# lightec-xyz/bls-verify-gadget

Measured on AMD Instinct MI355X. Metric: BLS-verify witness instances/sec (full pairing circuit), higher is better.
Workload: dtype u32 (381-bit Montgomery integers mod the BLS12-381 prime as 12 x 32-bit limbs in memory, products on 14 x 28-bit limbs with 64-bit columns; SHA-256 words)

## Files before the change

### __graft_entry__.py

```python
import importlib
import os
import subprocess
import sys

ROOT = os.path.dirname(os.path.abspath(__file__))
if ROOT not in sys.path:
    sys.path.insert(0, ROOT)


def build():
    pkg = importlib.import_module("bls-verify-gadget_amd")
    pkg.build(force=False)
    subprocess.check_call(["make", "-s", "-C", os.path.join(ROOT, "oracle")])
    subprocess.check_call(["make", "-s", "-C", os.path.join(ROOT, "tests", "hostsim")])
    subprocess.check_call(["make", "-s", "-C", os.path.join(ROOT, "tests", "vgroups")])
    subprocess.check_call(["make", "-s", "-j3", "-C", os.path.join(ROOT, "tests", "devfield")])
    subprocess.check_call(["make", "-s", "-C", os.path.join(ROOT, "tests", "msg_input")])
    subprocess.check_call(["make", "-s", "-C", os.path.join(ROOT, "tests", "agg_inputs")])
    subprocess.check_call(["make", "-s", "-C", os.path.join(ROOT, "tests", "c_caller")])
    subprocess.check_call(["make", "-s", "-C", os.path.join(ROOT, "tests", "cpp_caller")])
    pkg.lib()
    for s in pkg.EXPORTED_SYMBOLS:
        getattr(pkg.lib(), s)


def smoke():
    import numpy as np
    import torch

    from tests import oracle_lib, synth

    pkg = importlib.import_module("bls-verify-gadget_amd")
    o = oracle_lib.load()
    n = 4
    pk, msg, sig, expect = synth.make_batch(o, n, seed=0x5EED)
    dev = torch.device("cuda:0")
    g = pkg.BlsSignatureVerifyGadget(n, 32, device=dev)
    res = g.verify(pkg.ParametersVar(), pkg.PublicKeyVar.new_witness(torch.from_numpy(pk.view(np.int64)).to(dev)),
                   torch.from_numpy(msg).to(dev), pkg.SignatureVar.new_witness(torch.from_numpy(sig.view(np.int64)).to(dev)))
    torch.cuda.synchronize()
    got = res.cpu().numpy().astype(bool)
    w = g.witness.cpu().numpy().view(np.uint64)
    for i in range(n):
        nw, _, r, ow = o.witness(pk[i], msg[i].tobytes(), sig[i])
        assert r == bool(got[i]) == bool(expect[i]), (i, r, got[i], expect[i])
        assert nw == w.shape[1] and np.array_equal(ow, w[i]), "witness mismatch for instance %d" % i
    print("smoke ok: %d instances, %d witnesses each, bit-exact vs oracle" % (n, w.shape[1]))


if __name__ == "__main__":
    build()
    if "--smoke" in sys.argv:
        smoke()
```

### bls-verify-gadget_amd/csrc/fp.hpp

```cpp
#pragma once
#include <stdint.h>

#if defined(__HIPCC__)
#include <hip/hip_runtime.h>
#define BLSW_HD __host__ __device__ __forceinline__
#define BLSW_HD_NOINLINE inline __host__ __device__ __noinline__
#if defined(BLSW_INLINE_CHAINS) && defined(__HIP_DEVICE_COMPILE__)
#define BLSW_FN __host__ __device__ __forceinline__
#else
#define BLSW_FN inline __host__ __device__ __noinline__
#endif
#else
#define BLSW_HD inline
#define BLSW_HD_NOINLINE inline
#define BLSW_FN inline
#endif

namespace blsw {

struct Fp {
    uint32_t l[12];
};
struct Fp2 {
    Fp c0, c1;
// ... 29 lines not shown
    Fp r;
#pragma unroll
    for (int i = 0; i < 12; i++) r.l[i] = 0;
    return r;
}
BLSW_HD Fp fp_one() {
    constexpr uint32_t R1[12] = BLSW_R1_LIMBS;
    Fp r;
#pragma unroll
    for (int i = 0; i < 12; i++) r.l[i] = R1[i];
    return r;
}
BLSW_HD bool fp_is_zero(const Fp& a) {
    uint32_t o = 0;
#pragma unroll
    for (int i = 0; i < 12; i++) o |= a.l[i];
    return o == 0;
}
BLSW_HD bool fp_eq(const Fp& a, const Fp& b) {
    uint32_t o = 0;
#pragma unroll
    for (int i = 0; i < 12; i++) o |= a.l[i] ^ b.l[i];
    return o == 0;
}
#if defined(__clang__)
BLSW_HD uint32_t addc32(uint32_t a, uint32_t b, uint32_t& carry) {
    unsigned co;
    uint32_t r = __builtin_addc(a, b, carry, &co);
    carry = co;
    return r;
}
BLSW_HD uint32_t subb32(uint32_t a, uint32_t b, uint32_t& borrow) {
    unsigned bo;
    uint32_t r = __builtin_subc(a, b, borrow, &bo);
    borrow = bo;
    return r;
}
#else
BLSW_HD uint32_t addc32(uint32_t a, uint32_t b, uint32_t& carry) {
    uint64_t x = (uint64_t)a + b + carry;
    carry = (uint32_t)(x >> 32);
    return (uint32_t)x;
}
BLSW_HD uint32_t subb32(uint32_t a, uint32_t b, uint32_t& borrow) {
    uint64_t x = (uint64_t)a - b - borrow;
    borrow = (uint32_t)(x >> 32) & 1u;
    return (uint32_t)x;
}
#endif
BLSW_HD Fp fp_cond_sub_p(const Fp& a, uint32_t top) {
    constexpr uint32_t P[12] = BLSW_P_LIMBS;
    Fp d;
    uint32_t borrow = 0;
#pragma unroll
    for (int i = 0; i < 12; i++) d.l[i] = subb32(a.l[i], P[i], borrow);
    bool ge = (top != 0) || (borrow == 0);
    Fp r;
#pragma unroll
    for (int i = 0; i < 12; i++) r.l[i] = ge ? d.l[i] : a.l[i];
    return r;
}
BLSW_HD Fp fp_add(const Fp& a, const Fp& b) {
    Fp s;
    uint32_t c = 0;
#pragma unroll
    for (int i = 0; i < 12; i++) s.l[i] = addc32(a.l[i], b.l[i], c);
    return fp_cond_sub_p(s, c);
}
BLSW_HD Fp fp_sub(const Fp& a, const Fp& b) {
    constexpr uint32_t P[12] = BLSW_P_LIMBS;
    Fp d;
    uint32_t borrow = 0;
#pragma unroll
    for (int i = 0; i < 12; i++) d.l[i] = subb32(a.l[i], b.l[i], borrow);
    uint32_t mask = 0u - borrow;
    uint32_t c = 0;
    Fp r;
#pragma unroll
    for (int i = 0; i < 12; i++) r.l[i] = addc32(d.l[i], P[i] & mask, c);
    return r;
}
BLSW_HD Fp fp_neg(const Fp& a) { return fp_sub(fp_zero(), a); }
BLSW_HD Fp fp_dbl(const Fp& a) { return fp_add(a, a); }

#if defined(__HIPCC__)
typedef uint4 blsw_u4;
#else
struct blsw_u4 {
    uint32_t x, y, z, w;
};
#endif
BLSW_HD_NOINLINE Fp fp_mul_v(blsw_u4 a0, blsw_u4 a1, blsw_u4 a2, blsw_u4 b0, blsw_u4 b1, blsw_u4 b2) {
    constexpr uint32_t P[12] = BLSW_P_LIMBS;
    const uint32_t al[12] = {a0.x, a0.y, a0.z, a0.w, a1.x, a1.y, a1.z, a1.w, a2.x, a2.y, a2.z, a2.w};
    const uint32_t bl[12] = {b0.x, b0.y, b0.z, b0.w, b1.x, b1.y, b1.z, b1.w, b2.x, b2.y, b2.z, b2.w};
    uint32_t t[13];
#pragma unroll
    for (int i = 0; i < 13; i++) t[i] = 0;
#pragma unroll
    for (int i = 0; i < 12; i++) {
        const uint32_t bi = bl[i];
        uint64_t x[12];
#pragma unroll
        for (int j = 0; j < 12; j++) x[j] = (uint64_t)al[j] * bi + t[j];
        uint32_t c = 0;
        t[0] = (uint32_t)x[0];
#pragma unroll
        for (int j = 1; j < 12; j++) t[j] = addc32((uint32_t)x[j], (uint32_t)(x[j - 1] >> 32), c);
        t[12] = addc32(t[12], (uint32_t)(x[11] >> 32), c);
        const uint32_t m = t[0] * BLSW_INV32;
#pragma unroll
        for (int j = 0; j < 12; j++) x[j] = (uint64_t)m * P[j] + t[j];
        c = 0;
#pragma unroll
        for (int j = 1; j < 12; j++) t[j - 1] = addc32((uint32_t)x[j], (uint32_t)(x[j - 1] >> 32), c);
        t[11] = addc32(t[12], (uint32_t)(x[11] >> 32), c);
        t[12] = c;
    }
    Fp r;
#pragma unroll
    for (int i = 0; i < 12; i++) r.l[i] = t[i];
    return fp_cond_sub_p(r, 0);
}
#define BLSW_P28                                                                                                                               \
    {                                                                                                                                          \
        0xfffaaabu, 0xfefffffu, 0x3ffffb9u, 0xfffeb15u, 0x6241eabu, 0xa0f6b0fu, 0xf6730d2u, 0xf38512bu, 0x4774b84u, 0x4bacd76u, 0xba7b643u, \
            0xe69a4b1u, 0x1ea397fu, 0x001a011u                                                                                                 \
    }
#define BLSW_PINV28 0xffcfffdu
BLSW_HD_NOINLINE Fp fp_mul_v28(blsw_u4 a0, blsw_u4 a1, blsw_u4 a2, blsw_u4 b0, blsw_u4 b1, blsw_u4 b2) {
    constexpr uint32_t P28[14] = BLSW_P28;
    const uint32_t M28 = 0x0fffffffu;
    const uint32_t al[12] = {a0.x, a0.y, a0.z, a0.w, a1.x, a1.y, a1.z, a1.w, a2.x, a2.y, a2.z, a2.w};
    const uint32_t bl[12] = {b0.x, b0.y, b0.z, b0.w, b1.x, b1.y, b1.z, b1.w, b2.x, b2.y, b2.z, b2.w};
    uint32_t A[14], B[14];
#pragma unroll
    for (int i = 0; i < 14; i++) {
        const int bp = 28 * i, w = bp >> 5, sh = bp & 31;
        uint32_t v = al[w] >> sh;
        if (sh > 4 && w + 1 < 12) v |= al[w + 1] << (32 - sh);
        A[i] = v & M28;
        const int bq = 28 * i - 8;
        uint32_t u;
        if (bq < 0)
            u = bl[0] << 8;
        else {
            const int wq = bq >> 5, sq = bq & 31;
            u = bl[wq] >> sq;
            if (sq > 4 && wq + 1 < 12) u |= bl[wq + 1] << (32 - sq);
        }
        B[i] = u & M28;
    }
    uint64_t t[15];
#pragma unroll
    for (int j = 0; j < 15; j++) t[j] = 0;
#pragma unroll
    for (int i = 0; i < 14; i++) {
        const uint32_t bi = B[i];
#pragma unroll
        for (int j = 0; j < 14; j++) t[j] += (uint64_t)A[j] * bi;
        const uint32_t m = ((uint32_t)t[0] * BLSW_PINV28) & M28;
#pragma unroll
        for (int j = 0; j < 14; j++) t[j] += (uint64_t)m * P28[j];
        t[1] += t[0] >> 28;
#pragma unroll
        for (int j = 0; j < 14; j++) t[j] = t[j + 1];
// ... 324 lines not shown
```

### bls-verify-gadget_amd/csrc/team.hpp

```cpp
#pragma once
#include "team_tables.hpp"
#include "tower.hpp"

namespace blsw {

#if defined(__HIP_DEVICE_COMPILE__)
typedef uint32_t team_u32x4 __attribute__((ext_vector_type(4)));
typedef __attribute__((address_space(3))) team_u32x4 team_lds_u32x4;
BLSW_HD Fp2 team_ld(const Fp2* slots, uint32_t s) {
    const team_lds_u32x4* p = (const team_lds_u32x4*)(slots + s);
    team_u32x4 v0 = p[0], v1 = p[1], v2 = p[2], v3 = p[3], v4 = p[4], v5 = p[5];
    Fp2 r;
    r.c0.l[0] = v0.x; r.c0.l[1] = v0.y; r.c0.l[2] = v0.z; r.c0.l[3] = v0.w;
    r.c0.l[4] = v1.x; r.c0.l[5] = v1.y; r.c0.l[6] = v1.z; r.c0.l[7] = v1.w;
    r.c0.l[8] = v2.x; r.c0.l[9] = v2.y; r.c0.l[10] = v2.z; r.c0.l[11] = v2.w;
    r.c1.l[0] = v3.x; r.c1.l[1] = v3.y; r.c1.l[2] = v3.z; r.c1.l[3] = v3.w;
    r.c1.l[4] = v4.x; r.c1.l[5] = v4.y; r.c1.l[6] = v4.z; r.c1.l[7] = v4.w;
    r.c1.l[8] = v5.x; r.c1.l[9] = v5.y; r.c1.l[10] = v5.z; r.c1.l[11] = v5.w;
    return r;
}
BLSW_HD void team_st(Fp2* slots, uint32_t s, const Fp2& v) {
    team_lds_u32x4* p = (team_lds_u32x4*)(slots + s);
    p[0] = team_u32x4{v.c0.l[0], v.c0.l[1], v.c0.l[2], v.c0.l[3]};
    p[1] = team_u32x4{v.c0.l[4], v.c0.l[5], v.c0.l[6], v.c0.l[7]};
    p[2] = team_u32x4{v.c0.l[8], v.c0.l[9], v.c0.l[10], v.c0.l[11]};
    p[3] = team_u32x4{v.c1.l[0], v.c1.l[1], v.c1.l[2], v.c1.l[3]};
    p[4] = team_u32x4{v.c1.l[4], v.c1.l[5], v.c1.l[6], v.c1.l[7]};
    p[5] = team_u32x4{v.c1.l[8], v.c1.l[9], v.c1.l[10], v.c1.l[11]};
}
#else
BLSW_HD Fp2 team_ld(const Fp2* slots, uint32_t s) { return slots[s]; }
BLSW_HD void team_st(Fp2* slots, uint32_t s, const Fp2& v) { slots[s] = v; }
#endif

BLSW_HD uint32_t team_lin_idx(const TeamLin& L, uint32_t k) {
    uint64_t lo = L.idx[0] | ((uint64_t)L.idx[1] << 32), hi = L.idx[2] | ((uint64_t)L.idx[3] << 32);
    uint64_t w = (k & 8) ? hi : lo;
    return (uint32_t)(w >> ((k & 7) * 8)) & 0xffu;
}
BLSW_HD Fp2 team_gather(const TeamLin& L, const Fp2* slots) {
    Fp2 acc = fp2_zero();
    uint32_t k = 0;
    const uint32_t n0 = L.n & 0x3f, n1 = (L.n >> 8) & 0xff, n2 = (L.n >> 16) & 0xff, n3 = L.n >> 24;
    const uint32_t mscale = (L.n >> 6) & 3;
    if (n0) {
        acc = team_ld(slots, team_lin_idx(L, 0));
        k = 1;
        for (; k < n0; k++) acc = fp2_add(acc, team_ld(slots, team_lin_idx(L, k)));
    }
    for (uint32_t e = k + n1; k < e; k++) acc = fp2_sub(acc, team_ld(slots, team_lin_idx(L, k)));
    if (n2 + n3) {
        Fp2 m = fp2_zero();
        for (uint32_t e = k + n2; k < e; k++) m = fp2_add(m, team_ld(slots, team_lin_idx(L, k)));
        for (uint32_t e = k + n3; k < e; k++) m = fp2_sub(m, team_ld(slots, team_lin_idx(L, k)));
        if (mscale) {
            Fp2 m3 = fp2_add(fp2_dbl(m), m);
            Fp2 m12 = fp2_dbl(fp2_dbl(m3));
            m = mscale == 2 ? fp2_dbl(m12) : m12;
        }
        acc = fp2_add(acc, fp2_mul_xi(m));
    }
    return acc;
}

BLSW_HD void team_task(const TeamTask& t, Fp2* slots, const Emitter& e) {
    const uint32_t kind = t.hdr & 0xff, dst = (t.hdr >> 8) & 0xff;
    if (kind == TK_NONE) return;
    Fp2 a = team_gather(t.a, slots), b = team_gather(t.b, slots);
    Emitter w = e;
    w.pos += t.hdr >> 16;
    if (kind == TK_K3V || kind == TK_K2V) w.base = nullptr;
    Fp2 r = fp2_zero();
    if (kind == TK_K3 || kind == TK_K3V || kind == TK_K2S) {
        const bool sq = kind == TK_K2S;
        const Fp sum = fp_add(a.c0, a.c1), dif = fp_sub(a.c0, a.c1), bsum = fp_add(b.c0, b.c1);
        Fp y0, x1, y1;
#pragma unroll
        for (int i = 0; i < 12; i++) {
            y0.l[i] = sq ? a.c1.l[i] : b.c0.l[i];
            x1.l[i] = sq ? dif.l[i] : a.c1.l[i];
            y1.l[i] = sq ? sum.l[i] : b.c1.l[i];
        }
        Fp p0 = fp_mul(a.c0, y0), p1 = fp_mul(x1, y1);
        Fp p2 = fp_mul(sum, bsum);
        w.put(p0);
        w.put(p1);
        if (!sq) w.put(p2);
        Fp2 rk = {fp_sub(p0, p1), fp_sub(fp_sub(p2, p0), p1)};
        Fp2 rs = {p1, fp_dbl(p0)};
#pragma unroll
        for (int i = 0; i < 12; i++) {
            r.c0.l[i] = sq ? rs.c0.l[i] : rk.c0.l[i];
            r.c1.l[i] = sq ? rs.c1.l[i] : rk.c1.l[i];
        }
    } else if (kind == TK_K2 || kind == TK_K2V || kind == TK_K2B) {
        const bool sep = kind == TK_K2B;
        Fp x1 = fp_add(a.c0, a.c1);
#pragma unroll
        for (int i = 0; i < 12; i++) x1.l[i] = sep ? a.c1.l[i] : x1.l[i];
        Fp v0 = fp_mul(a.c0, b.c0);
        Fp s = fp_mul(x1, b.c0);
        w.put(v0);
        w.put(s);
        Fp d = fp_sub(s, v0);
#pragma unroll
        for (int i = 0; i < 12; i++) d.l[i] = sep ? s.l[i] : d.l[i];
        r = {v0, d};
    } else {
        w.put(fp_mul(a.c1, b.c1));
    }
    if (dst != 0xff) team_st(slots, dst, r);
}

BLSW_HD Fp2 team_conj(uint32_t j, const Fp2& v) { return j >= 3 ? fp2_neg(v) : v; }
BLSW_FN Fp2 team_frob(uint32_t j, const Fp2& v, int power) {
    Fp2 x = (power & 1) ? fp2_conj(v) : v;
    const uint32_t k = j % 3;
    Fp2 c6 = fp2_one();
    if (k == 1) c6 = power == 1 ? K_FROB6_C1_1() : (power == 2 ? K_FROB6_C1_2() : K_FROB6_C1_3());
    if (k == 2) c6 = power == 1 ? K_FROB6_C2_1() : (power == 2 ? K_FROB6_C2_2() : K_FROB6_C2_3());
    if (k != 0) x = fp2_mul(x, c6);
    if (j >= 3) x = fp2_mul(x, power == 1 ? K_FROB12_C1_1() : (power == 2 ? K_FROB12_C1_2() : K_FROB12_C1_3()));
    return x;
}
BLSW_HD bool team_is_one_coeff(uint32_t j, const Fp2& v, const Emitter& e_one) {
    Emitter w = e_one;
    w.pos += (j / 3) * 17 + (j % 3) * 5;
    return fp2_is_eq_w(w, j == 0 ? fp2_one() : fp2_zero(), v);
}
BLSW_HD bool team_is_one_tree(uint32_t j, const bool* b, const Emitter& e_one) {
    bool t0 = b[0] && b[1], r0 = t0 && b[2], t1 = b[3] && b[4], r1 = t1 && b[5];
    bool res = r0 && r1;
    Emitter w = e_one;
    if (j == 0) {
        w.pos += 15;
        w.put_bool(t0);
        w.put_bool(r0);
        w.pos = e_one.pos + 34;
        w.put_bool(res);
    } else if (j == 3) {
        w.pos += 17 + 15;
        w.put_bool(t1);
        w.put_bool(r1);
    }
    return res;
}
BLSW_FN void team_inverse_lane0(Fp2* slots) {
    Fp12 a = {{team_ld(slots, TS_IN0 + 0), team_ld(slots, TS_IN0 + 1), team_ld(slots, TS_IN0 + 2)},
              {team_ld(slots, TS_IN0 + 3), team_ld(slots, TS_IN0 + 4), team_ld(slots, TS_IN0 + 5)}};
    Fp12 inv = fp12_inv(a);
    team_st(slots, TS_IN1 + 0, inv.c0.c0);
    team_st(slots, TS_IN1 + 1, inv.c0.c1);
    team_st(slots, TS_IN1 + 2, inv.c0.c2);
    team_st(slots, TS_IN1 + 3, inv.c1.c0);
    team_st(slots, TS_IN1 + 4, inv.c1.c1);
    team_st(slots, TS_IN1 + 5, inv.c1.c2);
}
BLSW_HD Fp2 team_first_f(uint32_t j, const Fp2* slots) {
    if (j == 0) return team_ld(slots, TS_XS0);
    if (j == 1) return team_ld(slots, TS_XS1);
    if (j == 4) return team_ld(slots, TS_XYC);
    return fp2_zero();
}
BLSW_HD Fp2 team_first_f_var(uint32_t j, const Fp2* slots, const Emitter& e) {
    if (j == 0) return team_ld(slots, TS_XH0);
    if (j == 1) {
        const Fp2 c1 = team_ld(slots, TS_XH1);
        const Fp px = team_ld(slots, TS_XPX).c0;
        Fp2 r = {fp_mul(c1.c0, px), fp_mul(c1.c1, px)};
        Emitter w = e;
        w.put(r.c0);
        w.put(r.c1);
        return r;
    }
    if (j == 4) return team_ld(slots, TS_XYV);
    return fp2_zero();
}
template <class C>
BLSW_HD void team_load_coeff_lane(uint32_t j, Fp2* slots, const C& coeff_sig, const C& coeff_h, uint32_t k) {
    if (j == 0) team_st(slots, TS_XS0, {coeff_sig.ld(4 * k + 0), coeff_sig.ld(4 * k + 1)});
// ... 263 lines not shown
```

### bls-verify-gadget_amd/csrc/team_tables.hpp

```cpp
#pragma once
#include <stdint.h>
namespace blsw {
enum { TK_NONE = 0, TK_K3 = 1, TK_K3V = 2, TK_K2 = 3, TK_K2V = 4, TK_K2B = 5, TK_K1E = 6, TK_K2S = 7 };
enum { TS_IN0 = 0, TS_IN1 = 6, TS_P = 12, TS_XS0 = 30, TS_XS1 = 31, TS_XH0 = 32, TS_XH1 = 33, TS_XYC = 34, TS_XYV = 35, TS_XPX = 36, TS_NSLOTS = 37 };
enum { TEAM_MAX_TERMS = 16, TEAM_MAX_ROUNDS = 4 };
struct TeamLin { uint32_t n; uint32_t idx[4]; };
struct TeamTask { uint32_t hdr; TeamLin a, b; };
struct TeamOp { uint32_t rounds, n_witness; TeamTask task[TEAM_MAX_ROUNDS][6]; TeamLin out[6]; };
#if defined(__HIPCC__)
#define BLSW_TEAM_TABLE __constant__ const
#else
#define BLSW_TEAM_TABLE static const
#endif
BLSW_TEAM_TABLE TeamOp TEAM_OP_MUL = {3, 54, {
    {{0x00000c01u, {0x00000001u, {0x00000000u, 0x00000000u, 0x00000000u, 0x00000000u}}, {0x00000001u, {0x00000006u, 0x00000000u, 0x00000000u, 0x00000000u}}},
     {0x00030d01u, {0x00000001u, {0x00000001u, 0x00000000u, 0x00000000u, 0x00000000u}}, {0x00000001u, {0x00000007u, 0x00000000u, 0x00000000u, 0x00000000u}}},
     {0x00060e01u, {0x00000001u, {0x00000002u, 0x00000000u, 0x00000000u, 0x00000000u}}, {0x00000001u, {0x00000008u, 0x00000000u, 0x00000000u, 0x00000000u}}},
     {0x00090f01u, {0x00000002u, {0x00000201u, 0x00000000u, 0x00000000u, 0x00000000u}}, {0x00000002u, {0x00000807u, 0x00000000u, 0x00000000u, 0x00000000u}}},
     {0x000c1001u, {0x00000002u, {0x00000100u, 0x00000000u, 0x00000000u, 0x00000000u}}, {0x00000002u, {0x00000706u, 0x00000000u, 0x00000000u, 0x00000000u}}},
     {0x000f1101u, {0x00000002u, {0x00000200u, 0x00000000u, 0x00000000u, 0x00000000u}}, {0x00000002u, {0x00000806u, 0x00000000u, 0x00000000u, 0x00000000u}}}},
    {{0x00121201u, {0x00000001u, {0x00000003u, 0x00000000u, 0x00000000u, 0x00000000u}}, {0x00000001u, {0x00000009u, 0x00000000u, 0x00000000u, 0x00000000u}}},
     {0x00151301u, {0x00000001u, {0x00000004u, 0x00000000u, 0x00000000u, 0x00000000u}}, {0x00000001u, {0x0000000au, 0x00000000u, 0x00000000u, 0x00000000u}}},
     {0x00181401u, {0x00000001u, {0x00000005u, 0x00000000u, 0x00000000u, 0x00000000u}}, {0x00000001u, {0x0000000bu, 0x00000000u, 0x00000000u, 0x00000000u}}},
     {0x001b1501u, {0x00000002u, {0x00000504u, 0x00000000u, 0x00000000u, 0x00000000u}}, {0x00000002u, {0x00000b0au, 0x00000000u, 0x00000000u, 0x00000000u}}},
     {0x001e1601u, {0x00000002u, {0x00000403u, 0x00000000u, 0x00000000u, 0x00000000u}}, {0x00000002u, {0x00000a09u, 0x00000000u, 0x00000000u, 0x00000000u}}},
     {0x00211701u, {0x00000002u, {0x00000503u, 0x00000000u, 0x00000000u, 0x00000000u}}, {0x00000002u, {0x00000b09u, 0x00000000u, 0x00000000u, 0x00000000u}}}},
    {{0x00241801u, {0x00000002u, {0x00000300u, 0x00000000u, 0x00000000u, 0x00000000u}}, {0x00000002u, {0x00000906u, 0x00000000u, 0x00000000u, 0x00000000u}}},
     {0x00271901u, {0x00000002u, {0x00000401u, 0x00000000u, 0x00000000u, 0x00000000u}}, {0x00000002u, {0x00000a07u, 0x00000000u, 0x00000000u, 0x00000000u}}},
     {0x002a1a01u, {0x00000002u, {0x00000502u, 0x00000000u, 0x00000000u, 0x00000000u}}, {0x00000002u, {0x00000b08u, 0x00000000u, 0x00000000u, 0x00000000u}}},
     {0x002d1b01u, {0x00000004u, {0x05040201u, 0x00000000u, 0x00000000u, 0x00000000u}}, {0x00000004u, {0x0b0a0807u, 0x00000000u, 0x00000000u, 0x00000000u}}},
     {0x00301c01u, {0x00000004u, {0x04030100u, 0x00000000u, 0x00000000u, 0x00000000u}}, {0x00000004u, {0x0a090706u, 0x00000000u, 0x00000000u, 0x00000000u}}},
     {0x00331d01u, {0x00000004u, {0x05030200u, 0x00000000u, 0x00000000u, 0x00000000u}}, {0x00000004u, {0x0b090806u, 0x00000000u, 0x00000000u, 0x00000000u}}}},
    {{0x0000ff00u, {0x00000000u, {0x00000000u, 0x00000000u, 0x00000000u, 0x00000000u}}, {0x00000000u, {0x00000000u, 0x00000000u, 0x00000000u, 0x00000000u}}},
     {0x0000ff00u, {0x00000000u, {0x00000000u, 0x00000000u, 0x00000000u, 0x00000000u}}, {0x00000000u, {0x00000000u, 0x00000000u, 0x00000000u, 0x00000000u}}},
     {0x0000ff00u, {0x00000000u, {0x00000000u, 0x00000000u, 0x00000000u, 0x00000000u}}, {0x00000000u, {0x00000000u, 0x00000000u, 0x00000000u, 0x00000000u}}},
     {0x0000ff00u, {0x00000000u, {0x00000000u, 0x00000000u, 0x00000000u, 0x00000000u}}, {0x00000000u, {0x00000000u, 0x00000000u, 0x00000000u, 0x00000000u}}},
     {0x0000ff00u, {0x00000000u, {0x00000000u, 0x00000000u, 0x00000000u, 0x00000000u}}, {0x00000000u, {0x00000000u, 0x00000000u, 0x00000000u, 0x00000000u}}},
     {0x0000ff00u, {0x00000000u, {0x00000000u, 0x00000000u, 0x00000000u, 0x00000000u}}, {0x00000000u, {0x00000000u, 0x00000000u, 0x00000000u, 0x00000000u}}}},
  }, {{0x04030001u, {0x17130f0cu, 0x14120e0du, 0x00000000u, 0x00000000u}},
      {0x02020202u, {0x0d0c1210u, 0x1413150eu, 0x00000000u, 0x00000000u}},
      {0x00010403u, {0x0c16110du, 0x1413120eu, 0x00000000u, 0x00000000u}},
      {0x04050201u, {0x0d120c18u, 0x1b14130eu, 0x1a19150fu, 0x00000000u}},
      {0x02010405u, {0x13120d0cu, 0x1816101cu, 0x140e1a19u, 0x00000000u}},
      {0x00000606u, {0x14120e0cu, 0x110d1d19u, 0x1a181713u, 0x00000000u}}}};
BLSW_TEAM_TABLE TeamOp TEAM_OP_SQR = {2, 36, {
    {{0x00000c01u, {0x00000001u, {0x00000000u, 0x00000000u, 0x00000000u, 0x00000000u}}, {0x00000001u, {0x00000003u, 0x00000000u, 0x00000000u, 0x00000000u}}},
     {0x00030d01u, {0x00000001u, {0x00000001u, 0x00000000u, 0x00000000u, 0x00000000u}}, {0x00000001u, {0x00000004u, 0x00000000u, 0x00000000u, 0x00000000u}}},
     {0x00060e01u, {0x00000001u, {0x00000002u, 0x00000000u, 0x00000000u, 0x00000000u}}, {0x00000001u, {0x00000005u, 0x00000000u, 0x00000000u, 0x00000000u}}},
     {0x00090f01u, {0x00000002u, {0x00000201u, 0x00000000u, 0x00000000u, 0x00000000u}}, {0x00000002u, {0x00000504u, 0x00000000u, 0x00000000u, 0x00000000u}}},
     {0x000c1001u, {0x00000002u, {0x00000100u, 0x00000000u, 0x00000000u, 0x00000000u}}, {0x00000002u, {0x00000403u, 0x00000000u, 0x00000000u, 0x00000000u}}},
     {0x000f1101u, {0x00000002u, {0x00000200u, 0x00000000u, 0x00000000u, 0x00000000u}}, {0x00000002u, {0x00000503u, 0x00000000u, 0x00000000u, 0x00000000u}}}},
    {{0x00121201u, {0x00000101u, {0x00000300u, 0x00000000u, 0x00000000u, 0x00000000u}}, {0x01000001u, {0x00000500u, 0x00000000u, 0x00000000u, 0x00000000u}}},
     {0x00151301u, {0x00000101u, {0x00000401u, 0x00000000u, 0x00000000u, 0x00000000u}}, {0x00000101u, {0x00000301u, 0x00000000u, 0x00000000u, 0x00000000u}}},
     {0x00181401u, {0x00000101u, {0x00000502u, 0x00000000u, 0x00000000u, 0x00000000u}}, {0x00000101u, {0x00000402u, 0x00000000u, 0x00000000u, 0x00000000u}}},
     {0x001b1501u, {0x00000202u, {0x05040201u, 0x00000000u, 0x00000000u, 0x00000000u}}, {0x00000202u, {0x04030201u, 0x00000000u, 0x00000000u, 0x00000000u}}},
     {0x001e1601u, {0x00000202u, {0x04030100u, 0x00000000u, 0x00000000u, 0x00000000u}}, {0x01000102u, {0x05030100u, 0x00000000u, 0x00000000u, 0x00000000u}}},
     {0x00211701u, {0x00000202u, {0x05030200u, 0x00000000u, 0x00000000u, 0x00000000u}}, {0x01000102u, {0x05040200u, 0x00000000u, 0x00000000u, 0x00000000u}}}},
    {{0x0000ff00u, {0x00000000u, {0x00000000u, 0x00000000u, 0x00000000u, 0x00000000u}}, {0x00000000u, {0x00000000u, 0x00000000u, 0x00000000u, 0x00000000u}}},
     {0x0000ff00u, {0x00000000u, {0x00000000u, 0x00000000u, 0x00000000u, 0x00000000u}}, {0x00000000u, {0x00000000u, 0x00000000u, 0x00000000u, 0x00000000u}}},
     {0x0000ff00u, {0x00000000u, {0x00000000u, 0x00000000u, 0x00000000u, 0x00000000u}}, {0x00000000u, {0x00000000u, 0x00000000u, 0x00000000u, 0x00000000u}}},
     {0x0000ff00u, {0x00000000u, {0x00000000u, 0x00000000u, 0x00000000u, 0x00000000u}}, {0x00000000u, {0x00000000u, 0x00000000u, 0x00000000u, 0x00000000u}}},
     {0x0000ff00u, {0x00000000u, {0x00000000u, 0x00000000u, 0x00000000u, 0x00000000u}}, {0x00000000u, {0x00000000u, 0x00000000u, 0x00000000u, 0x00000000u}}},
     {0x0000ff00u, {0x00000000u, {0x00000000u, 0x00000000u, 0x00000000u, 0x00000000u}}, {0x00000000u, {0x00000000u, 0x00000000u, 0x00000000u, 0x00000000u}}}},
    {{0x0000ff00u, {0x00000000u, {0x00000000u, 0x00000000u, 0x00000000u, 0x00000000u}}, {0x00000000u, {0x00000000u, 0x00000000u, 0x00000000u, 0x00000000u}}},
     {0x0000ff00u, {0x00000000u, {0x00000000u, 0x00000000u, 0x00000000u, 0x00000000u}}, {0x00000000u, {0x00000000u, 0x00000000u, 0x00000000u, 0x00000000u}}},
     {0x0000ff00u, {0x00000000u, {0x00000000u, 0x00000000u, 0x00000000u, 0x00000000u}}, {0x00000000u, {0x00000000u, 0x00000000u, 0x00000000u, 0x00000000u}}},
     {0x0000ff00u, {0x00000000u, {0x00000000u, 0x00000000u, 0x00000000u, 0x00000000u}}, {0x00000000u, {0x00000000u, 0x00000000u, 0x00000000u, 0x00000000u}}},
     {0x0000ff00u, {0x00000000u, {0x00000000u, 0x00000000u, 0x00000000u, 0x00000000u}}, {0x00000000u, {0x00000000u, 0x00000000u, 0x00000000u, 0x00000000u}}},
     {0x0000ff00u, {0x00000000u, {0x00000000u, 0x00000000u, 0x00000000u, 0x00000000u}}, {0x00000000u, {0x00000000u, 0x00000000u, 0x00000000u, 0x00000000u}}}},
  }, {{0x05030002u, {0x110f120cu, 0x0e0e0c15u, 0x00001413u, 0x00000000u}},
      {0x01020302u, {0x120d1610u, 0x0d140f13u, 0x00000000u, 0x00000000u}},
      {0x00010504u, {0x17131110u, 0x120e0c0cu, 0x00000e14u, 0x00000000u}},
      {0x04020002u, {0x0f0f0c0cu, 0x0e0e0d0du, 0x00000000u, 0x00000000u}},
      {0x00020402u, {0x0c0c1010u, 0x0e0e0d0du, 0x00000000u, 0x00000000u}},
      {0x00000404u, {0x11110d0du, 0x0e0e0c0cu, 0x00000000u, 0x00000000u}}}};
BLSW_TEAM_TABLE TeamOp TEAM_OP_CYC = {1, 18, {
    {{0x00000c01u, {0x00000001u, {0x00000000u, 0x00000000u, 0x00000000u, 0x00000000u}}, {0x00000001u, {0x00000004u, 0x00000000u, 0x00000000u, 0x00000000u}}},
     {0x00030d01u, {0x00000002u, {0x00000400u, 0x00000000u, 0x00000000u, 0x00000000u}}, {0x00010001u, {0x00000400u, 0x00000000u, 0x00000000u, 0x00000000u}}},
     {0x00060e01u, {0x00000001u, {0x00000003u, 0x00000000u, 0x00000000u, 0x00000000u}}, {0x00000001u, {0x00000002u, 0x00000000u, 0x00000000u, 0x00000000u}}},
     {0x00090f01u, {0x00000002u, {0x00000302u, 0x00000000u, 0x00000000u, 0x00000000u}}, {0x00010001u, {0x00000203u, 0x00000000u, 0x00000000u, 0x00000000u}}},
     {0x000c1001u, {0x00000001u, {0x00000001u, 0x00000000u, 0x00000000u, 0x00000000u}}, {0x00000001u, {0x00000005u, 0x00000000u, 0x00000000u, 0x00000000u}}},
     {0x000f1101u, {0x00000002u, {0x00000501u, 0x00000000u, 0x00000000u, 0x00000000u}}, {0x00010001u, {0x00000501u, 0x00000000u, 0x00000000u, 0x00000000u}}}},
    {{0x0000ff00u, {0x00000000u, {0x00000000u, 0x00000000u, 0x00000000u, 0x00000000u}}, {0x00000000u, {0x00000000u, 0x00000000u, 0x00000000u, 0x00000000u}}},
     {0x0000ff00u, {0x00000000u, {0x00000000u, 0x00000000u, 0x00000000u, 0x00000000u}}, {0x00000000u, {0x00000000u, 0x00000000u, 0x00000000u, 0x00000000u}}},
     {0x0000ff00u, {0x00000000u, {0x00000000u, 0x00000000u, 0x00000000u, 0x00000000u}}, {0x00000000u, {0x00000000u, 0x00000000u, 0x00000000u, 0x00000000u}}},
     {0x0000ff00u, {0x00000000u, {0x00000000u, 0x00000000u, 0x00000000u, 0x00000000u}}, {0x00000000u, {0x00000000u, 0x00000000u, 0x00000000u, 0x00000000u}}},
     {0x0000ff00u, {0x00000000u, {0x00000000u, 0x00000000u, 0x00000000u, 0x00000000u}}, {0x00000000u, {0x00000000u, 0x00000000u, 0x00000000u, 0x00000000u}}},
     {0x0000ff00u, {0x00000000u, {0x00000000u, 0x00000000u, 0x00000000u, 0x00000000u}}, {0x00000000u, {0x00000000u, 0x00000000u, 0x00000000u, 0x00000000u}}}},
    {{0x0000ff00u, {0x00000000u, {0x00000000u, 0x00000000u, 0x00000000u, 0x00000000u}}, {0x00000000u, {0x00000000u, 0x00000000u, 0x00000000u, 0x00000000u}}},
     {0x0000ff00u, {0x00000000u, {0x00000000u, 0x00000000u, 0x00000000u, 0x00000000u}}, {0x00000000u, {0x00000000u, 0x00000000u, 0x00000000u, 0x00000000u}}},
     {0x0000ff00u, {0x00000000u, {0x00000000u, 0x00000000u, 0x00000000u, 0x00000000u}}, {0x00000000u, {0x00000000u, 0x00000000u, 0x00000000u, 0x00000000u}}},
// ... 234 lines not shown
```

Measured before the change: 130,200.

## Use lazy-reduction accumulators for team linear gathers and Karatsuba sums

Replaces the per-term modular add/sub chain in team_gather with a 13-word accumulator that is offset by a multiple of p, sums or subtracts all terms without reduction, multiplies by the xi scale directly, and performs a single Barrett-style reduction at the end. This applies to longer gathers or ones with an xi part. It also switches the Karatsuba pre-sums in team_task to lazy add/sub without a conditional subtraction, relying on the multiplier tolerating inputs above p. Bound constants are recorded in static_asserts, and correctness depends on those bounds and on the multiplier's input headroom.

```diff
diff --git a/__graft_entry__.py b/__graft_entry__.py
--- a/__graft_entry__.py
+++ b/__graft_entry__.py
@@ -15,6 +15,7 @@
     subprocess.check_call(["make", "-s", "-C", os.path.join(ROOT, "tests", "hostsim")])
     subprocess.check_call(["make", "-s", "-C", os.path.join(ROOT, "tests", "vgroups")])
     subprocess.check_call(["make", "-s", "-j3", "-C", os.path.join(ROOT, "tests", "devfield")])
+    subprocess.check_call(["make", "-s", "-j2", "-C", os.path.join(ROOT, "tests", "teamops")])
     subprocess.check_call(["make", "-s", "-C", os.path.join(ROOT, "tests", "msg_input")])
     subprocess.check_call(["make", "-s", "-C", os.path.join(ROOT, "tests", "agg_inputs")])
     subprocess.check_call(["make", "-s", "-C", os.path.join(ROOT, "tests", "c_caller")])
diff --git a/bls-verify-gadget_amd/csrc/fp.hpp b/bls-verify-gadget_amd/csrc/fp.hpp
--- a/bls-verify-gadget_amd/csrc/fp.hpp
+++ b/bls-verify-gadget_amd/csrc/fp.hpp
@@ -135,6 +135,88 @@
 }
 BLSW_HD Fp fp_neg(const Fp& a) { return fp_sub(fp_zero(), a); }
 BLSW_HD Fp fp_dbl(const Fp& a) { return fp_add(a, a); }
+BLSW_HD Fp fp_add_lazy(const Fp& a, const Fp& b) {
+    Fp s;
+    uint32_t c = 0;
+#pragma unroll
+    for (int i = 0; i < 12; i++) s.l[i] = addc32(a.l[i], b.l[i], c);
+    return s;
+}
+BLSW_HD Fp fp_sub_lazy(const Fp& a, const Fp& b) {
+    constexpr uint32_t P[12] = BLSW_P_LIMBS;
+    Fp d, r;
+    uint32_t borrow = 0, c = 0;
+#pragma unroll
+    for (int i = 0; i < 12; i++) d.l[i] = subb32(a.l[i], b.l[i], borrow);
+#pragma unroll
+    for (int i = 0; i < 12; i++) r.l[i] = addc32(d.l[i], P[i], c);
+    return r;
+}
+
+struct FpAcc {
+    uint32_t l[12];
+    uint32_t top;
+};
+#define BLSW_FPACC_MU 0x2760u
+#define BLSW_FPACC_MAX_WEIGHT 1024u
+constexpr FpAcc fpacc_const_kp(uint32_t k) {
+    constexpr uint32_t P[12] = BLSW_P_LIMBS;
+    FpAcc r{};
+    uint64_t c = 0;
+    for (int i = 0; i < 12; i++) {
+        c += (uint64_t)P[i] * k;
+        r.l[i] = (uint32_t)c;
+        c >>= 32;
+    }
+    r.top = (uint32_t)c;
+    return r;
+}
+template <uint32_t K>
+BLSW_HD FpAcc fpacc_kp() {
+    constexpr FpAcc c = fpacc_const_kp(K);
+    FpAcc r;
+#pragma unroll
+    for (int i = 0; i < 12; i++) r.l[i] = c.l[i];
+    r.top = c.top;
+    return r;
+}
+BLSW_HD void fpacc_add(FpAcc& a, const Fp& b) {
+    uint32_t c = 0;
+#pragma unroll
+    for (int i = 0; i < 12; i++) a.l[i] = addc32(a.l[i], b.l[i], c);
+    a.top += c;
+}
+BLSW_HD void fpacc_sub(FpAcc& a, const Fp& b) {
+    uint32_t borrow = 0;
+#pragma unroll
+    for (int i = 0; i < 12; i++) a.l[i] = subb32(a.l[i], b.l[i], borrow);
+    a.top -= borrow;
+}
+BLSW_HD void fpacc_mul_small(FpAcc& a, uint32_t m) {
+    uint64_t c = 0;
+#pragma unroll
+    for (int i = 0; i < 12; i++) {
+        c += (uint64_t)a.l[i] * m;
+        a.l[i] = (uint32_t)c;
+        c >>= 32;
+    }
+    a.top = a.top * m + (uint32_t)c;
+}
+BLSW_HD Fp fpacc_reduce(const FpAcc& a) {
+    constexpr uint32_t P[12] = BLSW_P_LIMBS;
+    const uint32_t x = (a.top << 8) | (a.l[11] >> 24);
+    const uint32_t q = (x * BLSW_FPACC_MU) >> 18;
+    Fp r;
+    uint64_t c = 0;
+    uint32_t borrow = 0;
+#pragma unroll
+    for (int i = 0; i < 12; i++) {
+        c += (uint64_t)P[i] * q;
+        r.l[i] = subb32(a.l[i], (uint32_t)c, borrow);
+        c >>= 32;
+    }
+    return fp_cond_sub_p(r, 0);
+}
 
 #if defined(__HIPCC__)
 typedef uint4 blsw_u4;
diff --git a/bls-verify-gadget_amd/csrc/team.hpp b/bls-verify-gadget_amd/csrc/team.hpp
--- a/bls-verify-gadget_amd/csrc/team.hpp
+++ b/bls-verify-gadget_amd/csrc/team.hpp
@@ -19,6 +19,15 @@
     r.c1.l[8] = v5.x; r.c1.l[9] = v5.y; r.c1.l[10] = v5.z; r.c1.l[11] = v5.w;
     return r;
 }
+BLSW_HD Fp team_ld_half(const Fp2* slots, uint32_t s, uint32_t comp) {
+    const team_lds_u32x4* p = (const team_lds_u32x4*)(slots + s) + 3 * comp;
+    team_u32x4 v0 = p[0], v1 = p[1], v2 = p[2];
+    Fp r;
+    r.l[0] = v0.x; r.l[1] = v0.y; r.l[2] = v0.z; r.l[3] = v0.w;
+    r.l[4] = v1.x; r.l[5] = v1.y; r.l[6] = v1.z; r.l[7] = v1.w;
+    r.l[8] = v2.x; r.l[9] = v2.y; r.l[10] = v2.z; r.l[11] = v2.w;
+    return r;
+}
 BLSW_HD void team_st(Fp2* slots, uint32_t s, const Fp2& v) {
     team_lds_u32x4* p = (team_lds_u32x4*)(slots + s);
     p[0] = team_u32x4{v.c0.l[0], v.c0.l[1], v.c0.l[2], v.c0.l[3]};
@@ -30,6 +39,7 @@
 }
 #else
 BLSW_HD Fp2 team_ld(const Fp2* slots, uint32_t s) { return slots[s]; }
+BLSW_HD Fp team_ld_half(const Fp2* slots, uint32_t s, uint32_t comp) { return comp ? slots[s].c1 : slots[s].c0; }
 BLSW_HD void team_st(Fp2* slots, uint32_t s, const Fp2& v) { slots[s] = v; }
 #endif
 
@@ -38,29 +48,57 @@
     uint64_t w = (k & 8) ? hi : lo;
     return (uint32_t)(w >> ((k & 7) * 8)) & 0xffu;
 }
-BLSW_HD Fp2 team_gather(const TeamLin& L, const Fp2* slots) {
+BLSW_HD Fp2 team_gather_short(const TeamLin& L, const Fp2* slots, uint32_t n0, uint32_t n1) {
     Fp2 acc = fp2_zero();
     uint32_t k = 0;
-    const uint32_t n0 = L.n & 0x3f, n1 = (L.n >> 8) & 0xff, n2 = (L.n >> 16) & 0xff, n3 = L.n >> 24;
-    const uint32_t mscale = (L.n >> 6) & 3;
     if (n0) {
         acc = team_ld(slots, team_lin_idx(L, 0));
         k = 1;
         for (; k < n0; k++) acc = fp2_add(acc, team_ld(slots, team_lin_idx(L, k)));
     }
     for (uint32_t e = k + n1; k < e; k++) acc = fp2_sub(acc, team_ld(slots, team_lin_idx(L, k)));
-    if (n2 + n3) {
-        Fp2 m = fp2_zero();
-        for (uint32_t e = k + n2; k < e; k++) m = fp2_add(m, team_ld(slots, team_lin_idx(L, k)));
-        for (uint32_t e = k + n3; k < e; k++) m = fp2_sub(m, team_ld(slots, team_lin_idx(L, k)));
+    return acc;
+}
+enum { TEAM_ACC_OFFSET = 16 };
+static_assert((int)TEAM_ACC_OFFSET >= (int)TEAM_LIN_BORROW_C0 && (int)TEAM_ACC_OFFSET >= (int)TEAM_LIN_BORROW_C1, "the accumulator's offset must cover every subtracted element");
+static_assert((uint32_t)TEAM_LIN_MAX_SCALE * TEAM_ACC_OFFSET + TEAM_LIN_POS_C0 < BLSW_FPACC_MAX_WEIGHT && (uint32_t)TEAM_LIN_MAX_SCALE * TEAM_ACC_OFFSET + TEAM_LIN_POS_C1 < BLSW_FPACC_MAX_WEIGHT,
+              "scaled offset + positive weight must stay below the bound fpacc_reduce's single conditional subtraction is proved for");
+template <int PHASE>
+BLSW_HD void team_acc_phase(FpAcc& c0, FpAcc& c1, const TeamLin& L, const Fp2* slots, uint32_t k, uint32_t n) {
+    if (n == 0) return;
+    const uint32_t last = k + n - 1;
+    Fp h0 = team_ld_half(slots, team_lin_idx(L, k), 0);
+    for (; k <= last; k++) {
+        const Fp h1 = team_ld_half(slots, team_lin_idx(L, k), 1);
+        if (PHASE == 0 || PHASE == 2) fpacc_add(c0, h0);
+        if (PHASE == 1 || PHASE == 3) fpacc_sub(c0, h0);
+        if (PHASE == 2) fpacc_add(c1, h0);
+        if (PHASE == 3) fpacc_sub(c1, h0);
+        const Fp nx = team_ld_half(slots, team_lin_idx(L, k < last ? k + 1 : last), 0);
+        if (PHASE == 0 || PHASE == 2) fpacc_add(c1, h1);
+        if (PHASE == 1 || PHASE == 3) fpacc_sub(c1, h1);
+        if (PHASE == 2) fpacc_sub(c0, h1);
+        if (PHASE == 3) fpacc_add(c0, h1);
+        h0 = nx;
+    }
+}
+BLSW_HD Fp2 team_gather(const TeamLin& L, const Fp2* slots) {
+    const uint32_t n0 = L.n & 0x3f, n1 = (L.n >> 8) & 0xff, n2 = (L.n >> 16) & 0xff, n3 = L.n >> 24;
+    const uint32_t mscale = (L.n >> 6) & 3;
+    if (BLSW_WAVE_ANY(n0 + n1 + n2 + n3 > 3 || n2 + n3 != 0)) {
+        FpAcc c0 = fpacc_kp<TEAM_ACC_OFFSET>(), c1 = fpacc_kp<TEAM_ACC_OFFSET>();
+        team_acc_phase<2>(c0, c1, L, slots, n0 + n1, n2);
+        team_acc_phase<3>(c0, c1, L, slots, n0 + n1 + n2, n3);
         if (mscale) {
-            Fp2 m3 = fp2_add(fp2_dbl(m), m);
-            Fp2 m12 = fp2_dbl(fp2_dbl(m3));
-            m = mscale == 2 ? fp2_dbl(m12) : m12;
-        }
-        acc = fp2_add(acc, fp2_mul_xi(m));
-    }
-    return acc;
+            const uint32_t m = mscale == 2 ? 24u : 12u;
+            fpacc_mul_small(c0, m);
+            fpacc_mul_small(c1, m);
+        }
+        team_acc_phase<0>(c0, c1, L, slots, 0, n0);
+        team_acc_phase<1>(c0, c1, L, slots, n0, n1);
+        return {fpacc_reduce(c0), fpacc_reduce(c1)};
+    }
+    return team_gather_short(L, slots, n0, n1);
 }
 
 BLSW_HD void team_task(const TeamTask& t, Fp2* slots, const Emitter& e) {
@@ -73,7 +111,7 @@
     Fp2 r = fp2_zero();
     if (kind == TK_K3 || kind == TK_K3V || kind == TK_K2S) {
         const bool sq = kind == TK_K2S;
-        const Fp sum = fp_add(a.c0, a.c1), dif = fp_sub(a.c0, a.c1), bsum = fp_add(b.c0, b.c1);
+        const Fp sum = fp_add_lazy(a.c0, a.c1), dif = fp_sub_lazy(a.c0, a.c1), bsum = fp_add_lazy(b.c0, b.c1);
         Fp y0, x1, y1;
 #pragma unroll
         for (int i = 0; i < 12; i++) {
@@ -95,7 +133,7 @@
         }
     } else if (kind == TK_K2 || kind == TK_K2V || kind == TK_K2B) {
         const bool sep = kind == TK_K2B;
-        Fp x1 = fp_add(a.c0, a.c1);
+        Fp x1 = fp_add_lazy(a.c0, a.c1);
 #pragma unroll
         for (int i = 0; i < 12; i++) x1.l[i] = sep ? a.c1.l[i] : x1.l[i];
         Fp v0 = fp_mul(a.c0, b.c0);
diff --git a/bls-verify-gadget_amd/csrc/team_tables.hpp b/bls-verify-gadget_amd/csrc/team_tables.hpp
--- a/bls-verify-gadget_amd/csrc/team_tables.hpp
+++ b/bls-verify-gadget_amd/csrc/team_tables.hpp
@@ -7,6 +7,7 @@
 struct TeamLin { uint32_t n; uint32_t idx[4]; };
 struct TeamTask { uint32_t hdr; TeamLin a, b; };
 struct TeamOp { uint32_t rounds, n_witness; TeamTask task[TEAM_MAX_ROUNDS][6]; TeamLin out[6]; };
+enum { TEAM_LIN_POS_C0 = 36, TEAM_LIN_NEG_C0 = 36, TEAM_LIN_BORROW_C0 = 11, TEAM_LIN_POS_C1 = 48, TEAM_LIN_NEG_C1 = 48, TEAM_LIN_BORROW_C1 = 11, TEAM_LIN_MAX_SCALE = 24 };
 #if defined(__HIPCC__)
 #define BLSW_TEAM_TABLE __constant__ const
 #else
```

Measured after the change: 127,100. -2.4%, worse.
